# emtiyaz/vmp-for-svae

Measured on AMD Instinct MI355X. Metric: vmp_step_datapoints_per_sec, higher is better.
Workload: dtype f32

## Files before the change

### vmp-for-svae_amd/csrc/vmp_mix.hip

```cpp
#include "vmp_common.h"
#include "vmp_linalg.h"
#include <stdlib.h>
#include <type_traits>

using namespace vmp;

namespace {

constexpr int TR = 64;
constexpr int LS = 68;
constexpr int MAX_NW = 8;
constexpr int MAX_NW1 = 8;
constexpr int max_nw(int KT) { return KT == 1 ? MAX_NW1 : MAX_NW; }
constexpr int MAX_BLOCKS = 1024;

struct PassArgs {
    const float* x;
    const float* r_in;
    const float* u_in;
    const uint8_t* mask;
    const float* pivot;
    const float* pack;
    float* r_out;
    float* u_out;
    float* logr_out;
    double* partials;
    long long N;
    long long rpw;
    long long rpw_b;
    int K;
    int vec_ok;
    int par_reduce;
#ifdef VMP_DEBUG_TS
    long long* dbg_t;
#endif
};
#ifdef VMP_DEBUG_TS
#define PASS_TS(i) do { if (a.dbg_t && (blockIdx.x == 0 || blockIdx.x == 100) && (threadIdx.x & 63) == 0) { a.dbg_t[(blockIdx.x ? 64 : 0) + (threadIdx.x >> 6) * 8 + (i)] = clock64(); \
    if ((i) == 0 && threadIdx.x == 0) a.dbg_t[(blockIdx.x ? 64 : 0) + 7] = wall_clock64();           \
    if ((i) == 5 && threadIdx.x == 64) a.dbg_t[(blockIdx.x ? 64 : 0) + 8 + 7] = wall_clock64(); } } while (0)
#else
#define PASS_TS(i) do { } while (0)
#endif

#define VMP_DPP2(OP, CTRL)                                                   \
    "v_" OP "_f32_dpp %0, %0, %0 " CTRL " row_mask:0xf bank_mask:0xf\n\t"  \
    "v_" OP "_f32_dpp %1, %1, %1 " CTRL " row_mask:0xf bank_mask:0xf\n\t"  \
    "s_nop 0\n\t"
#define VMP_DPP2_FIRST(OP, CTRL)                                             \
    "v_" OP "_f32_dpp %0, %2, %2 " CTRL " row_mask:0xf bank_mask:0xf\n\t"  \
    "v_" OP "_f32_dpp %1, %3, %3 " CTRL " row_mask:0xf bank_mask:0xf\n\t"  \
    "s_nop 0\n\t"
__device__ __forceinline__ v2f row16_max2(v2f v) {
    float a, b;
    asm("s_nop 1\n\t" VMP_DPP2_FIRST("max", "row_ror:8") VMP_DPP2("max", "row_ror:4") VMP_DPP2("max", "row_ror:2")
        VMP_DPP2("max", "row_ror:1")
        : "=&v"(a), "=&v"(b) : "v"(v.x), "v"(v.y));
    return v2f{a, b};
}
__device__ __forceinline__ v2f row16_sum2(v2f v) {
    float a, b;
    asm("s_nop 1\n\t" VMP_DPP2_FIRST("add", "row_ror:8") VMP_DPP2("add", "row_ror:4") VMP_DPP2("add", "row_ror:2")
        VMP_DPP2("add", "row_ror:1")
        : "=&v"(a), "=&v"(b) : "v"(v.x), "v"(v.y));
    return v2f{a, b};
}

constexpr int MOM_TERMS = 3;
#ifndef VMP_MOM_FLUSH
#define VMP_MOM_FLUSH 2
#endif

template <int D, int KT, int FLAV>
__device__ __forceinline__ void pass_epilogue(const PassArgs& a, float* smem, const double (&dacc)[KT][Geo<D>::FT][4],
                                              const double (&dn)[KT][4], int lane, int wave, int nw) {
    using G = Geo<D>;
    constexpr int FT = G::FT;
    constexpr bool SMM = (FLAV == VMP_SMM);
    const int K = a.K;
    {
        __syncthreads();
        PASS_TS(3);
        double* sc = reinterpret_cast<double*>(smem);
        constexpr int SLAB = KT * (FT + 1) * 4 * WAVE;
        if (a.par_reduce) {
            double* mine = sc + wave * SLAB;
#pragma unroll
            for (int kt = 0; kt < KT; ++kt)
#pragma unroll
                for (int c = 0; c < 4; ++c) {
#pragma unroll
                    for (int ft = 0; ft < FT; ++ft) mine[((kt * (FT + 1) + ft) * 4 + c) * WAVE + lane] = dacc[kt][ft][c];
                    mine[((kt * (FT + 1) + FT) * 4 + c) * WAVE + lane] = SMM ? dn[kt][c] : dacc[kt][0][c];
                }
            __syncthreads();
            constexpr int EPT = 2, NWB = max_nw(KT);
            for (int e0 = threadIdx.x; e0 < SLAB; e0 += EPT * blockDim.x) {
                double vals[EPT][NWB];
#pragma unroll
                for (int q = 0; q < EPT; ++q) {
                    const int e = e0 + q * blockDim.x;
#pragma unroll
                    for (int w = 0; w < NWB; ++w) vals[q][w] = (e < SLAB && w < nw) ? sc[w * SLAB + e] : 0.0;
                }
#pragma unroll
                for (int q = 0; q < EPT; ++q) {
                    const int e = e0 + q * blockDim.x;
                    double t2 = vals[q][0];
#pragma unroll
                    for (int w = 1; w < NWB; ++w) t2 += vals[q][w];
                    if (e < SLAB) sc[e] = t2;
                }
            }
            __syncthreads();
        } else {
            for (int w = 0; w < nw; ++w) {
                if (wave == w) {
#pragma unroll
                    for (int kt = 0; kt < KT; ++kt)
#pragma unroll
                        for (int c = 0; c < 4; ++c) {
#pragma unroll
                            for (int ft = 0; ft < FT; ++ft) {
                                const int idx = ((kt * (FT + 1) + ft) * 4 + c) * WAVE + lane;
                                sc[idx] = (w == 0 ? 0.0 : sc[idx]) + dacc[kt][ft][c];
                            }
                            const int idn = ((kt * (FT + 1) + FT) * 4 + c) * WAVE + lane;
                            sc[idn] = (w == 0 ? 0.0 : sc[idn]) + (SMM ? dn[kt][c] : dacc[kt][0][c]);
                        }
                }
                __syncthreads();
            }
        }
        PASS_TS(4);
        constexpr int PX = G::PF + 1;
        double* out = a.partials;
        for (int e = threadIdx.x; e < KT * (FT + 1) * 4 * WAVE; e += blockDim.x) {
            const int l = e & 63, c = (e >> 6) & 3, tf = (e >> 8) % (FT + 1), kt = (e >> 8) / (FT + 1);
            const int k = kt * 16 + (l >> 4) * 4 + c;
            if (k >= K) continue;
            double* row = out + ((long long)k * MAX_BLOCKS + blockIdx.x) * PX;
            if (tf < FT) {
                const int f = tf * 16 + (l & 15);
                if (f < G::F) row[f] = sc[e];
            } else if ((l & 15) == 0) {
                row[G::F] = sc[e];
            }
        }
        if (wave == 0) {
            double ntot = 0.0;
#pragma unroll
            for (int kt = 0; kt < KT; ++kt) {
                const int k = kt * 16 + (lane & 15), l = ((k & 15) >> 2) * 16, c = k & 3;
                const double nk = (lane < 16 && k < K) ? sc[((kt * (FT + 1) + FT) * 4 + c) * WAVE + l] : 0.0;
#pragma unroll
                for (int j = 0; j < 16; ++j) ntot += readlane_d(nk, j);
            }
            for (int k = lane; k < K; k += WAVE) out[((long long)k * MAX_BLOCKS + blockIdx.x) * PX + G::PF] = ntot;
        }
        PASS_TS(5);
    }
}

template <int D, int KT, int FLAV, bool ESTEP, bool STATS, bool MASK>
__global__ __launch_bounds__(max_nw(KT) * WAVE) void pass_kernel(PassArgs a) {
    using G = Geo<D>;
    constexpr int FT = G::FT;
    constexpr bool SMM = (FLAV == VMP_SMM);
    extern __shared__ __attribute__((aligned(16))) float smem[];

    const int lane = threadIdx.x & 63, wave = threadIdx.x >> 6, nw = blockDim.x >> 6;
    const int K = a.K;
    PASS_TS(0);
#ifdef VMP_DEBUG_TS
    if (a.dbg_t && (blockIdx.x == 0 || blockIdx.x == 100) && (threadIdx.x & 63) == 0)
        a.dbg_t[(blockIdx.x ? 64 : 0) + (threadIdx.x >> 6) * 8 + 6] = __builtin_amdgcn_s_getreg((31 << 11) | 4);
#endif
    float* xl = smem + wave * (G::XROWS * LS);
    constexpr int ONE = D, ZERO = D + 1;
    xl[ONE * LS + lane] = 1.0f;
    xl[ZERO * LS + lane] = 0.0f;
    const int ppos = (lane & ~7) + 2 * (lane & 3) + ((lane >> 2) & 1);

    const bool vec = a.vec_ok != 0;
    long long lo, hi;
    if (a.rpw_b == a.rpw) {
        lo = ((long long)blockIdx.x * nw + wave) * a.rpw;
        hi = lo + a.rpw;
    } else {
        const int hw = nw >> 1;
        const long long base = (long long)blockIdx.x * hw * (a.rpw + a.rpw_b);
        lo = wave < hw ? base + wave * a.rpw : base + hw * a.rpw + (wave - hw) * a.rpw_b;
        hi = lo + (wave < hw ? a.rpw : a.rpw_b);
    }
    if (hi > a.N) hi = a.N;
    float xr[D];
    {
        const long long n = lo + lane;
#pragma unroll
        for (int j = 0; j < D; ++j) xr[j] = 0.f;
        if (n < hi) load_row<D>(a.x + n * D, xr, vec);
    }
    const int i16 = lane & 15, kk = lane >> 4;
    float pv[D];
    {
        const float* __restrict__ pp = a.pivot ? a.pivot : a.x;
        const bool hasp = a.pivot != nullptr;
#pragma unroll
        for (int j = 0; j < D; ++j) { const float v = pp[j]; pv[j] = hasp ? v : 0.f; }
    }

    constexpr int MP = (D + 1) / 2, WP = (G::TRI + 1) / 2;
    v2f pm2[KT][MP], pw2[KT][WP], pch[KT];
    float pua[KT], pub[KT];
    if constexpr (ESTEP) {
#pragma unroll
        for (int kt = 0; kt < KT; ++kt) {
            const int k = kt * 16 + i16;
            const bool on = k < K;
// ... 234 lines not shown
#pragma unroll
                    for (int ft = 0; ft < FT; ++ft) {
                        split_bf16<MOM_TERMS>(fa[ft] * fb[ft], t3);
#pragma unroll
                        for (int t = 0; t < 3; ++t) Bs[ft][t][u] = t3[t];
                    }
                }
            };
            using std::integral_constant;
            const bool full = (K == 16 * KT) && (n0 + 32 <= trows);
            if (full) {
                group(integral_constant<bool, true>{}, integral_constant<int, 0>{});
                group(integral_constant<bool, true>{}, integral_constant<int, 1>{});
                group(integral_constant<bool, true>{}, integral_constant<int, 2>{});
                group(integral_constant<bool, true>{}, integral_constant<int, 3>{});
            } else {
                group(integral_constant<bool, false>{}, integral_constant<int, 0>{});
                group(integral_constant<bool, false>{}, integral_constant<int, 1>{});
                group(integral_constant<bool, false>{}, integral_constant<int, 2>{});
                group(integral_constant<bool, false>{}, integral_constant<int, 3>{});
            }

            if constexpr (STATS) {
                bf16x8 b[FT][3];
#pragma unroll
                for (int ft = 0; ft < FT; ++ft)
#pragma unroll
                    for (int t = 0; t < 3; ++t)
                        b[ft][t] = __builtin_bit_cast(bf16x8, u32x4{Bs[ft][t][0], Bs[ft][t][1], Bs[ft][t][2], Bs[ft][t][3]});
#pragma unroll
                for (int kt = 0; kt < KT; ++kt) {
                    bf16x8 av[3], rv[3];
#pragma unroll
                    for (int t = 0; t < 3; ++t) {
                        av[t] = __builtin_bit_cast(bf16x8, u32x4{As[kt][t][0], As[kt][t][1], As[kt][t][2], As[kt][t][3]});
                        if constexpr (SMM) rv[t] = __builtin_bit_cast(bf16x8, u32x4{Rs[kt][t][0], Rs[kt][t][1], Rs[kt][t][2], Rs[kt][t][3]});
                    }
#pragma unroll
                    for (int ta = 0; ta < MOM_TERMS; ++ta) {
#pragma unroll
                        for (int tb = 0; tb + ta < MOM_TERMS; ++tb) {
#pragma unroll
                            for (int ft = 0; ft < FT; ++ft) {
                                if (ta + tb == 0) acc[kt][ft] = __builtin_amdgcn_mfma_f32_16x16x32_bf16(av[ta], b[ft][tb], acc[kt][ft], 0, 0, 0);
                                else acs[kt][ft] = __builtin_amdgcn_mfma_f32_16x16x32_bf16(av[ta], b[ft][tb], acs[kt][ft], 0, 0, 0);
                            }
                        }
                        if constexpr (SMM) {
                            if (ta == 0) nacc[kt] = __builtin_amdgcn_mfma_f32_16x16x32_bf16(rv[ta], b[0][0], nacc[kt], 0, 0, 0);
                            else nacs[kt] = __builtin_amdgcn_mfma_f32_16x16x32_bf16(rv[ta], b[0][0], nacs[kt], 0, 0, 0);
                        }
                    }
                }
            }
        }

        if constexpr (STATS) {
            if (((row0 - lo) / TR) % VMP_MOM_FLUSH == VMP_MOM_FLUSH - 1 || row0 + TR >= hi) {
#pragma unroll
                for (int kt = 0; kt < KT; ++kt) {
#pragma unroll
                    for (int c = 0; c < 4; ++c) {
                        if constexpr (SMM) dn[kt][c] += (double)nacc[kt][c] + (double)nacs[kt][c];
#pragma unroll
                        for (int ft = 0; ft < FT; ++ft) dacc[kt][ft][c] += (double)acc[kt][ft][c] + (double)acs[kt][ft][c];
                    }
                    nacc[kt] = f32x4{0.f, 0.f, 0.f, 0.f};
                    nacs[kt] = f32x4{0.f, 0.f, 0.f, 0.f};
#pragma unroll
                    for (int ft = 0; ft < FT; ++ft) { acc[kt][ft] = f32x4{0.f, 0.f, 0.f, 0.f}; acs[kt][ft] = f32x4{0.f, 0.f, 0.f, 0.f}; }
                }
            }
        }
        __builtin_amdgcn_wave_barrier();
    }

    PASS_TS(2);
    if constexpr (STATS) pass_epilogue<D, KT, FLAV>(a, smem, dacc, dn, lane, wave, nw);
}


constexpr int AIS = 36;

struct FinArgs {
    const double* partials;
    const double* stats_in;
    int nblk, K, flavour, src, do_post;
    const float *alpha0, *beta0, *m0, *C0, *v0, *kappa;
    const float* pivot;
    float *alpha, *beta, *m, *C, *v, *xbar, *S, *pi, *pack;
    double* pack64;
    double* stats_out;
    double* peer[VMP_EXCH_MAX_RANKS];
    int nranks, rank;
    unsigned long long iter;
    int* status;
#ifdef VMP_DEBUG_TS
    long long* dbg_t;
#endif
};

#ifdef VMP_DEBUG_TS
#define FIN_TS(i) do { if (a.dbg_t && blockIdx.x == 0 && tid == 0) { a.dbg_t[i] = clock64(); if ((i) == 0) a.dbg_t[6] = wall_clock64(); if ((i) == 5) a.dbg_t[7] = wall_clock64(); } } while (0)
#else
#define FIN_TS(i) do { } while (0)
#endif

template <int D>
__device__ void finalize_block(const FinArgs& a, const int k, const int tid, const int nthreads);

template <int D> constexpr int xdl_wave_floats() { return Geo<D>::XROWS * LS + TR * AIS; }

template <int D, int FLAV, bool STATS, int MT = 3>
__device__ __forceinline__ void pass_xdl_body(const PassArgs& a) {
    using G = Geo<D>;
    constexpr int FT = G::FT, KT = 1;
    constexpr bool SMM = (FLAV == VMP_SMM);
    constexpr int DP = (D + 1) / 2;
    extern __shared__ __attribute__((aligned(16))) float smem[];
    const int lane = threadIdx.x & 63, wave = threadIdx.x >> 6, nw = blockDim.x >> 6;
    const int K = a.K;
    PASS_TS(0);
    float* xl = smem + wave * xdl_wave_floats<D>();
    unsigned* ai = reinterpret_cast<unsigned*>(xl + G::XROWS * LS);
    constexpr int ONE = D, ZERO = D + 1;
    const int ppos = (lane & ~15) + 4 * (lane & 3) + ((lane >> 2) & 3);

    const bool vec = a.vec_ok != 0;
    long long lo, hi;
    if (a.rpw_b == a.rpw) {
        lo = ((long long)blockIdx.x * nw + wave) * a.rpw;
        hi = lo + a.rpw;
    } else {
        const int hw = nw >> 1;
        const long long base = (long long)blockIdx.x * hw * (a.rpw + a.rpw_b);
        lo = wave < hw ? base + wave * a.rpw : base + hw * a.rpw + (wave - hw) * a.rpw_b;
        hi = lo + (wave < hw ? a.rpw : a.rpw_b);
    }
    if (hi > a.N) hi = a.N;
    float xr[D];
    {
        const long long n = lo + lane;
#pragma unroll
        for (int j = 0; j < D; ++j) xr[j] = 0.f;
        if (n < hi) load_row<D>(a.x + n * D, xr, vec);
    }
    const int i16 = lane & 15, kk = lane >> 4;
    float pv[D];
    {
        const float* __restrict__ pp = a.pivot ? a.pivot : a.x;
        const bool hasp = a.pivot != nullptr;
#pragma unroll
        for (int j = 0; j < D; ++j) { const float v = pp[j]; pv[j] = hasp ? v : 0.f; }
    }

    constexpr int NS = D < 4 ? D : 4;
    constexpr int NB = D > 4 ? D - 4 : 0;
    constexpr int QK = 3 * NS + 4 * NB, QS = QK | 1;
    static_assert(16 * QS * 4 <= xdl_wave_floats<D>(), "the operand image must fit the LDS of a one-wave launch");
    u32x4 Bsm[NS], B1[NB > 0 ? NB : 1], B2[NB > 0 ? NB : 1];
    v2f pch;
    float pua, pub;
    {
        const bool on = i16 < K;
        const float* __restrict__ pc = a.pack + (on ? i16 : 0) * G::PACK + D + G::TRI;
        const float c0 = pc[0], c1 = pc[1], c2 = pc[2], c3 = pc[3];
        pch.x = on ? c0 : -INFINITY;
        pch.y = on ? c1 : 0.f;
        pua = on ? c2 : 0.f;
        pub = on ? c3 : 1.f;
    }
    {
        u32x4* img = reinterpret_cast<u32x4*>(smem);
        for (int it = threadIdx.x; it < 16 * D; it += blockDim.x) {
            const int k = it / D, i = it - k * D;
            const bool on = k < K;
            const float* __restrict__ p = a.pack + (on ? k : 0) * G::PACK;
            const int tri = i * (i + 1) / 2;
            float mr[D], wr[D];
#pragma unroll
            for (int j = 0; j < D; ++j) { mr[j] = p[j]; wr[j] = p[D + tri + j]; }
            double bi = 0.0;
#pragma unroll
            for (int j = 0; j < D; ++j)
                if (j <= i) bi -= (double)wr[j] * ((double)mr[j] - (double)pv[j]);
            unsigned tb[3];
            split_bf16<3>(v2f{(float)bi, 0.f}, tb);
            const unsigned bias0 = (tb[0] & 0xffffu) | (tb[1] << 16), bias1 = tb[2] & 0xffffu;
            unsigned th[4] = {0u, 0u, 0u, 0u}, tm[4] = {0u, 0u, 0u, 0u}, tl[4] = {0u, 0u, 0u, 0u};
#pragma unroll
            for (int q = 0; q < DP; ++q) {
                const int j0 = 2 * q, j1 = 2 * q + 1;
                const float wa = j0 <= i ? wr[j0] : 0.f;
                const float wb = (j1 <= i && j1 < D) ? wr[j1 < D ? j1 : 0] : 0.f;
                unsigned t3[3];
                split_bf16<3>(v2f{wa, wb}, t3);
                th[q] = t3[0]; tm[q] = t3[1]; tl[q] = t3[2];
            }
            const u32x4 zero = u32x4{0u, 0u, 0u, 0u};
            const u32x4 bias = on ? u32x4{bias0, bias1, 0u, 0u} : zero;
            if (i < NS) {
                u32x4* o = img + k * QS + 3 * i;
                o[0] = on ? u32x4{th[0], th[1], tm[0], tm[1]} : zero;
                o[1] = on ? u32x4{th[0], th[1], tl[0], tl[1]} : zero;
                o[2] = bias;
            } else {
                u32x4* o = img + k * QS + 3 * NS + 4 * (i - 4);
                o[0] = on ? u32x4{th[0], th[1], th[2], th[3]} : zero;
                o[1] = on ? u32x4{tm[0], tm[1], tm[2], tm[3]} : zero;
                o[2] = on ? u32x4{tl[0], tl[1], tl[2], tl[3]} : zero;
                o[3] = bias;
            }
        }
        __syncthreads();
        const u32x4* q = img + i16 * QS;
        const int s0 = kk == 1 ? 1 : (kk == 3 ? 2 : 0);
#pragma unroll
        for (int i = 0; i < NS; ++i) Bsm[i] = q[3 * i + s0];
        if constexpr (NB > 0) {
            const int s1 = kk == 1 ? 3 : (kk == 2 ? 1 : 0), s2 = kk == 0 ? 2 : (kk == 1 ? 0 : 1);
#pragma unroll
            for (int ib = 0; ib < NB; ++ib) {
                B1[ib] = q[3 * NS + 4 * ib + s1];
                const u32x4 w2 = q[3 * NS + 4 * ib + s2];
                B2[ib] = kk == 3 ? u32x4{0u, 0u, 0u, 0u} : w2;
            }
        }
        __syncthreads();
    }
    xl[ONE * LS + lane] = 1.0f;
    xl[ZERO * LS + lane] = 0.0f;
    {
        u32x4 ones = u32x4{0x3F803F80u, 0x00003F80u, 0u, 0u}, zeros = u32x4{0u, 0u, 0u, 0u};
        *reinterpret_cast<u32x4*>(ai + lane * AIS + 12) = ones;
        *reinterpret_cast<u32x4*>(ai + lane * AIS + 16) = zeros;
    }
    const int rho = 4 * (i16 & 3) + (i16 >> 2);
    const int offA1 = rho * AIS + (kk == 1 ? 12 : (kk == 3 ? 4 : 0));
    const int offA2 = rho * AIS + (kk == 0 ? 0 : (kk == 1 ? 8 : (kk == 2 ? 4 : 16)));
    const int offA3 = rho * AIS + (kk == 3 ? 12 : 20 + 4 * kk);

    int offA[FT], offB[FT];
#pragma unroll
    for (int ft = 0; ft < FT; ++ft) {
        const int f = ft * 16 + i16;
        int ra = ZERO, rb = ZERO;
        if (f == 0) { ra = ONE; rb = ONE; }
        else if (f <= D) { ra = f - 1; rb = ONE; }
        else if (f < G::F) {
            int p = f - D - 1, d = 0;
            while (p >= D - d) { p -= D - d; ++d; }
            ra = d; rb = d + p;
        }
        offA[ft] = ra * LS + 4 * kk;
        offB[ft] = rb * LS + 4 * kk;
    }

    f32x4 acc[KT][FT], acs[KT][FT];
    double dacc[KT][FT][4];
    double dn[KT][4];
    float nsum = 0.f;
    double dnl = 0.0;
#pragma unroll
    for (int c = 0; c < 4; ++c) dn[0][c] = 0.0;
#pragma unroll
    for (int ft = 0; ft < FT; ++ft) {
        acc[0][ft] = f32x4{0.f, 0.f, 0.f, 0.f};
        acs[0][ft] = f32x4{0.f, 0.f, 0.f, 0.f};
#pragma unroll
        for (int c = 0; c < 4; ++c) dacc[0][ft][c] = 0.0;
    }

#ifdef VMP_DEBUG_TS
    asm volatile("" :: "v"(xr[0]), "v"(pv[0]), "v"(pch.x), "v"(Bsm[0][0]));
    asm volatile("s_waitcnt vmcnt(0)" ::: "memory");
#endif
    PASS_TS(1);
    for (long long row0 = lo; row0 < hi; row0 += TR) {
        const int trows = (hi - row0 < TR) ? (int)(hi - row0) : TR;
        {
            const bool valid = row0 + lane < hi;
            float xs[2 * DP];
#pragma unroll
            for (int j = 0; j < 2 * DP; ++j) xs[j] = (valid && j < D) ? xr[j < D ? j : 0] - pv[j < D ? j : 0] : 0.f;
#pragma unroll
            for (int j = 0; j < D; ++j) xl[j * LS + ppos] = xs[j];
            unsigned th[4] = {0u, 0u, 0u, 0u}, tm[4] = {0u, 0u, 0u, 0u}, tl[4] = {0u, 0u, 0u, 0u};
#pragma unroll
            for (int q = 0; q < DP; ++q) {
                unsigned t3[3];
                split_bf16<3>(v2f{xs[2 * q], xs[2 * q + 1]}, t3);
                th[q] = t3[0]; tm[q] = t3[1]; tl[q] = t3[2];
            }
            *reinterpret_cast<u32x4*>(ai + lane * AIS) = u32x4{th[0], th[1], th[2], th[3]};
            *reinterpret_cast<u32x4*>(ai + lane * AIS + 4) = u32x4{tm[0], tm[1], tm[2], tm[3]};
            *reinterpret_cast<u32x4*>(ai + lane * AIS + 8) = u32x4{tl[0], tl[1], tl[2], tl[3]};
            *reinterpret_cast<u32x4*>(ai + lane * AIS + 20) = u32x4{th[0], th[1], th[0], th[1]};
            *reinterpret_cast<u32x4*>(ai + lane * AIS + 24) = u32x4{tm[0], tm[1], th[0], th[1]};
            *reinterpret_cast<u32x4*>(ai + lane * AIS + 28) = u32x4{tl[0], tl[1], tm[0], tm[1]};
            const long long n2 = row0 + TR + lane;
#pragma unroll
            for (int j = 0; j < D; ++j) xr[j] = 0.f;
            if (n2 < hi) load_row<D>(a.x + n2 * D, xr, vec);
        }
        __builtin_amdgcn_wave_barrier();

        const long long tbase = (row0 + kk) * K + i16;
#pragma unroll 1
        for (int n0 = 0; n0 < trows; n0 += 32) {
            const bool full = (K == 16) && (n0 + 32 <= trows);
            auto body = [&](auto full_c) __attribute__((always_inline)) {
            constexpr bool FULL = decltype(full_c)::value;
            unsigned As[3][4], Bs[FT][3][4];
            auto subtile = [&](auto jj_c) __attribute__((always_inline)) {
                constexpr int jj = decltype(jj_c)::value;
                const int n16 = n0 + 16 * jj;
                if (!FULL && n16 >= trows) {
                    if constexpr (STATS) {
#pragma unroll
                        for (int t = 0; t < 3; ++t) {
                            As[t][2 * jj] = 0u; As[t][2 * jj + 1] = 0u;
#pragma unroll
                            for (int ft = 0; ft < FT; ++ft) { Bs[ft][t][2 * jj] = 0u; Bs[ft][t][2 * jj + 1] = 0u; }
                        }
                    }
                    return;
                }
                f32x4 y[D];
                {
                    const bf16x8 a3 = __builtin_bit_cast(bf16x8, *reinterpret_cast<const u32x4*>(ai + n16 * AIS + offA3));
#pragma unroll
                    for (int i = 0; i < NS; ++i)
                        y[i] = __builtin_amdgcn_mfma_f32_16x16x32_bf16(a3, __builtin_bit_cast(bf16x8, Bsm[i]), f32x4{0.f, 0.f, 0.f, 0.f}, 0, 0, 0);
                }
                if constexpr (NB > 0) {
                    const bf16x8 a1 = __builtin_bit_cast(bf16x8, *reinterpret_cast<const u32x4*>(ai + n16 * AIS + offA1));
                    const bf16x8 a2 = __builtin_bit_cast(bf16x8, *reinterpret_cast<const u32x4*>(ai + n16 * AIS + offA2));
#pragma unroll
                    for (int i = 0; i < NB; ++i)
                        y[4 + i] = __builtin_amdgcn_mfma_f32_16x16x32_bf16(a1, __builtin_bit_cast(bf16x8, B1[i]), f32x4{0.f, 0.f, 0.f, 0.f}, 0, 0, 0);
#pragma unroll
                    for (int i = 0; i < NB; ++i)
                        y[4 + i] = __builtin_amdgcn_mfma_f32_16x16x32_bf16(a2, __builtin_bit_cast(bf16x8, B2[i]), y[4 + i], 0, 0, 0);
                }
                f32x4 q4 = y[0] * y[0], q4b = f32x4{0.f, 0.f, 0.f, 0.f};
#pragma unroll
                for (int i = 1; i < D; ++i) {
                    if (i & 1) q4b = __builtin_elementwise_fma(y[i], y[i], q4b);
                    else q4 = __builtin_elementwise_fma(y[i], y[i], q4);
                }
                q4 += q4b;
                v2f lg[2], uu[2], rr[2], w[2];
#pragma unroll
                for (int h = 0; h < 2; ++h) {
                    const v2f qh = v2f{q4[2 * h], q4[2 * h + 1]};
                    lg[h] = pk_const_minus_scaled(qh, pch);
                    if constexpr (SMM) uu[h] = v2f{pua * __builtin_amdgcn_rcpf(qh.x + pub), pua * __builtin_amdgcn_rcpf(qh.y + pub)};
                }
#pragma unroll
                for (int h = 0; h < 2; ++h) {
                    const v2f mx = row16_max2(lg[h]);
                    lg[h] = v2f{__builtin_amdgcn_exp2f(lg[h].x - mx.x), __builtin_amdgcn_exp2f(lg[h].y - mx.y)};
                    const v2f ssum = row16_sum2(lg[h]);
                    v2f inv = v2f{__builtin_amdgcn_rcpf(ssum.x), __builtin_amdgcn_rcpf(ssum.y)};
                    if constexpr (!FULL) {
                        const bool va = row0 + n16 + 8 * h + kk < hi, vb = row0 + n16 + 8 * h + 4 + kk < hi;
                        inv = v2f{va ? inv.x : 0.f, vb ? inv.y : 0.f};
                    }
                    rr[h] = lg[h] * inv;
                    w[h] = SMM ? rr[h] * uu[h] : rr[h];
                }
#pragma unroll
                for (int v = 0; v < 4; ++v) {
                    const float rv = rr[v >> 1][v & 1];
                    if constexpr (FULL) {
                        float* __restrict__ ro = a.r_out + tbase + (long long)(n16 + 4 * v) * 16;
                        __builtin_nontemporal_store(rv, ro);
                        if constexpr (SMM) __builtin_nontemporal_store(uu[v >> 1][v & 1], a.u_out + tbase + (long long)(n16 + 4 * v) * 16);
                        if (a.logr_out) a.logr_out[tbase + (long long)(n16 + 4 * v) * 16] = logf(rv);
                    } else {
                        const bool sv = (row0 + n16 + 4 * v + kk < hi) && i16 < K;
                        const long long o = tbase + (long long)(n16 + 4 * v) * K;
                        if (sv) {
                            a.r_out[o] = rv;
                            if constexpr (SMM) a.u_out[o] = uu[v >> 1][v & 1];
                            if (a.logr_out) a.logr_out[o] = logf(rv);
                        }
                    }
                }
                if constexpr (STATS) {
                    unsigned t3[3];
#pragma unroll
                    for (int h = 0; h < 2; ++h) {
                        split_bf16<MT>(w[h], t3);
#pragma unroll
                        for (int t = 0; t < 3; ++t) As[t][2 * jj + h] = t3[t];
                    }
                    if constexpr (SMM) nsum += (rr[0].x + rr[0].y) + (rr[1].x + rr[1].y);
#pragma unroll
                    for (int ft = 0; ft < FT; ++ft) {
                        const f32x4 fa = *reinterpret_cast<const f32x4*>(&xl[offA[ft] + n16]);
                        const f32x4 fb = *reinterpret_cast<const f32x4*>(&xl[offB[ft] + n16]);
                        const f32x4 pr = fa * fb;
#pragma unroll
                        for (int h = 0; h < 2; ++h) {
                            split_bf16<MT>(v2f{pr[2 * h], pr[2 * h + 1]}, t3);
#pragma unroll
                            for (int t = 0; t < 3; ++t) Bs[ft][t][2 * jj + h] = t3[t];
                        }
                    }
                }
            };
            using std::integral_constant;
            subtile(integral_constant<int, 0>{});
            subtile(integral_constant<int, 1>{});

            if constexpr (STATS) {
                bf16x8 b[FT][3];
#pragma unroll
                for (int ft = 0; ft < FT; ++ft)
#pragma unroll
                    for (int t = 0; t < 3; ++t)
                        b[ft][t] = __builtin_bit_cast(bf16x8, u32x4{Bs[ft][t][0], Bs[ft][t][1], Bs[ft][t][2], Bs[ft][t][3]});
                bf16x8 av[3];
#pragma unroll
                for (int t = 0; t < 3; ++t) av[t] = __builtin_bit_cast(bf16x8, u32x4{As[t][0], As[t][1], As[t][2], As[t][3]});
#pragma unroll
                for (int ta = 0; ta < MT; ++ta) {
#pragma unroll
                    for (int tb = 0; tb + ta < MT; ++tb) {
#pragma unroll
                        for (int ft = 0; ft < FT; ++ft) {
                            if (ta + tb == 0) acc[0][ft] = __builtin_amdgcn_mfma_f32_16x16x32_bf16(av[ta], b[ft][tb], acc[0][ft], 0, 0, 0);
                            else acs[0][ft] = __builtin_amdgcn_mfma_f32_16x16x32_bf16(av[ta], b[ft][tb], acs[0][ft], 0, 0, 0);
                        }
                    }
                }
            }
            };
            if (full) body(std::integral_constant<bool, true>{});
            else body(std::integral_constant<bool, false>{});
        }

        if constexpr (STATS) {
            if (((row0 - lo) / TR) % VMP_MOM_FLUSH == VMP_MOM_FLUSH - 1 || row0 + TR >= hi) {
#pragma unroll
                for (int c = 0; c < 4; ++c) {
#pragma unroll
                    for (int ft = 0; ft < FT; ++ft) dacc[0][ft][c] += (double)acc[0][ft][c] + (double)acs[0][ft][c];
                }
                if constexpr (SMM) { dnl += (double)nsum; nsum = 0.f; }
#pragma unroll
                for (int ft = 0; ft < FT; ++ft) { acc[0][ft] = f32x4{0.f, 0.f, 0.f, 0.f}; acs[0][ft] = f32x4{0.f, 0.f, 0.f, 0.f}; }
            }
        }
        __builtin_amdgcn_wave_barrier();
    }

    PASS_TS(2);
    if constexpr (STATS && SMM) {
        double tot = dnl;
        {
            int lo = __double2loint(tot), hi = __double2hiint(tot);
            tot += __hiloint2double(__shfl_xor(hi, 32), __shfl_xor(lo, 32));
            lo = __double2loint(tot); hi = __double2hiint(tot);
            tot += __hiloint2double(__shfl_xor(hi, 16), __shfl_xor(lo, 16));
        }
#pragma unroll
        for (int c = 0; c < 4; ++c) {
            const int src = 4 * kk + c;
            const int lo = __shfl(__double2loint(tot), src), hi = __shfl(__double2hiint(tot), src);
            dn[0][c] = __hiloint2double(hi, lo);
        }
    }
    if constexpr (STATS) pass_epilogue<D, 1, FLAV>(a, smem, dacc, dn, lane, wave, nw);
}

template <int D, int FLAV, bool STATS, int MT = 3>
__global__ __launch_bounds__(MAX_NW1 * WAVE) void pass_xdl_kernel(PassArgs a) {
    pass_xdl_body<D, FLAV, STATS, MT>(a);
}

__device__ double digamma_d(double x) {
    double r = 0.0;
    while (x < 10.0) { r -= 1.0 / x; x += 1.0; }
    const double f = 1.0 / (x * x);
    return r + log(x) - 0.5 / x
           - f * (1.0 / 12 - f * (1.0 / 120 - f * (1.0 / 252 - f * (1.0 / 240 - f * (1.0 / 132 - f * (691.0 / 32760))))));
}

template <int D>
__device__ void write_pack(float* pack, int k, const double* m, const double* W ,
                           double c, double h, double ua, double ub) {
    using G = Geo<D>;
    float* p = pack + k * G::PACK;
    int idx = D;
    for (int j = 0; j < D; ++j) p[j] = (float)m[j];
    for (int i = 0; i < D; ++i)
        for (int j = 0; j <= i; ++j) p[idx++] = (float)W[i * D + j];
    const double LOG2E = 1.4426950408889634074;
    p[idx++] = (float)(c * LOG2E); p[idx++] = (float)(h * LOG2E); p[idx++] = (float)ua; p[idx++] = (float)ub;
}

__device__ __forceinline__ double fast_rsqrt_d(double x) {
    double y = __builtin_amdgcn_rsq(x);
    y = y * (1.5 - 0.5 * x * y * y);
    y = y * (1.5 - 0.5 * x * y * y);
    return y;
}

template <int D>
__device__ __forceinline__ void wave_chol_inverse(const double* A, int lane, double (&X)[D], double& sumlog, bool& ok) {
    double row[D], rd[D];
#pragma unroll
    for (int e = 0; e < D; ++e)
        row[e] = lane < D ? 0.5 * (A[lane * D + e] + A[e * D + lane]) : (e == lane ? 1.0 : 0.0);
    ok = true;
    double mydiag = 1.0;
#pragma unroll
    for (int j = 0; j < D; ++j) {
        double t = row[j];
#pragma unroll
        for (int p = 0; p < j; ++p) t -= row[p] * readlane_d(row[p], j);
        const double sj = readlane_d(t, j);
        ok = ok && (sj > 0.0);
        rd[j] = fast_rsqrt_d(sj);
        if (lane == j) mydiag = sj;
        row[j] = lane >= j ? t * rd[j] : 0.0;
    }
    double lg = lane < D ? 0.5 * log(mydiag) : 0.0;
    sumlog = 0.0;
#pragma unroll
    for (int j = 0; j < D; ++j) sumlog += readlane_d(lg, j);
#pragma unroll
    for (int i = 0; i < D; ++i) {
        double acc = (i == lane) ? 1.0 : 0.0;
#pragma unroll
        for (int p = 0; p < i; ++p) acc -= readlane_d(row[p], i) * X[p];
        X[i] = acc * rd[i];
    }
}

template <int D>
__device__ void estep_constants(int k, int flavour, double alpha_k, double alpha_sum, double beta_k, double v_k,
                                double logdetP, double kap, double& c, double& h, double& ua, double& ub, double& elp) {
    const double LOG2 = 0.69314718055994530942, PI = 3.14159265358979323846;
    elp = digamma_d(alpha_k) - digamma_d(alpha_sum);
    double sdg = 0.0;
    if (flavour == VMP_GMM) {
        for (int i = 0; i < D; ++i) sdg += digamma_d(0.5 * (v_k + 1.0 + i));
        const double ld = (logdetP > log(1e-20)) ? logdetP : 0.0;
        const double eld = sdg + D * LOG2 + ld;
        c = elp + 0.5 * eld - 0.5 * (D / beta_k);
        h = 0.5; ua = 1.0; ub = 1.0;
    } else {
        for (int i = 0; i < D; ++i) sdg += digamma_d(0.5 * (v_k + i));
        const double eld = sdg + D * LOG2 + logdetP;
        h = 0.5 * (D + kap);
        c = lgamma(0.5 * (D + kap)) - lgamma(0.5 * kap) - 0.5 * D * log(kap * PI) + elp + 0.5 * eld
            - h * (D / beta_k) + log(kap);
        ua = D + kap;
        ub = D / beta_k + kap;
    }
}

constexpr int FIN_THREADS = 1024;
constexpr int FIN_MAX_GROUPS = FIN_THREADS / 64;

__device__ __forceinline__ void st_pack(const FinArgs& a, int idx, double v) {
    a.pack[idx] = (float)v;
    if (a.pack64) a.pack64[idx] = v;
}

template <int D>
__device__ void finalize_block(const FinArgs& a, const int k, const int tid, const int nthreads) {
    using G = Geo<D>;
    __shared__ double part[FIN_MAX_GROUPS][64];
    __shared__ double st[G::SW];
    __shared__ double ntot;
    __shared__ double Ck[D * D], mk[D], sp[D + 4], scal[8];
    __shared__ double alpha0s[VMP_MAX_K];
    const int K = a.K;
    const int FIN_GROUPS = nthreads >> 6;
    const bool post = a.do_post != 0;
    const bool smm = a.flavour == VMP_SMM;
    const double beta0 = post ? (double)a.beta0[k] : 0.0, v0 = post ? (double)a.v0[k] : 0.0;
    const double alpha0 = post ? (double)a.alpha0[k] : 0.0;
    const double kap = (post && smm) ? (double)a.kappa[k] : 0.0;
    bool shifted = (a.src == 0) && (a.pivot != nullptr);
    double m0d = 0.0, m0e = 0.0, C0de = 0.0, cd = 0.0, ce = 0.0;
    if (tid < D * D) {
        const int d = tid / D, e = tid % D;
        if (post) { m0d = a.m0[k * D + d]; m0e = a.m0[k * D + e]; C0de = a.C0[(k * D + d) * D + e]; }
        if (shifted) { cd = a.pivot[d]; ce = a.pivot[e]; }
    }
    if (post && tid < K) alpha0s[tid] = a.alpha0[tid];

    FIN_TS(0);
    if (a.src == 0) {
        constexpr int PX = G::PF + 1;
        const int f = tid & 63, g = tid >> 6;
        const double* __restrict__ mine = a.partials + (long long)k * MAX_BLOCKS * PX;
        for (int lg = g; lg < FIN_MAX_GROUPS; lg += FIN_GROUPS) {
            double s = 0.0;
            for (int b0 = lg; b0 < a.nblk; b0 += FIN_MAX_GROUPS * 16) {
                double v1[16];
                const int fc = f < PX ? f : PX - 1;
#pragma unroll
                for (int i = 0; i < 16; ++i) {
// ... 845 lines not shown
```

Measured before the change: 21.18 billion.

## Add specialized full-tile K=16 loop with fused 4-wide DPP softmax reductions

Splits the row loop into a fast path for full 64-row tiles when K==16, where both 32-row sub-bodies are unrolled with compile-time offsets and stride, and a generic tail loop. In the fast path the softmax max and sum reductions over the two half-tiles are interleaved into single 4-register DPP sequences, so independent DPP ops fill each other's hazard slots. The logr store is moved out of the per-element store loop, and the pivot is made wave-uniform via readfirstlane. This adds code size and register pressure.

```diff
diff --git a/vmp-for-svae_amd/csrc/vmp_mix.hip b/vmp-for-svae_amd/csrc/vmp_mix.hip
--- a/vmp-for-svae_amd/csrc/vmp_mix.hip
+++ b/vmp-for-svae_amd/csrc/vmp_mix.hip
@@ -65,6 +65,37 @@
         : "=&v"(a), "=&v"(b) : "v"(v.x), "v"(v.y));
     return v2f{a, b};
 }
+
+#define VMP_DPP4(OP, CTRL)                                                   \
+    "v_" OP "_f32_dpp %0, %0, %0 " CTRL " row_mask:0xf bank_mask:0xf\n\t"  \
+    "v_" OP "_f32_dpp %1, %1, %1 " CTRL " row_mask:0xf bank_mask:0xf\n\t"  \
+    "v_" OP "_f32_dpp %2, %2, %2 " CTRL " row_mask:0xf bank_mask:0xf\n\t"  \
+    "v_" OP "_f32_dpp %3, %3, %3 " CTRL " row_mask:0xf bank_mask:0xf\n\t"
+#define VMP_DPP4_FIRST(OP, CTRL)                                             \
+    "v_" OP "_f32_dpp %0, %4, %4 " CTRL " row_mask:0xf bank_mask:0xf\n\t"  \
+    "v_" OP "_f32_dpp %1, %5, %5 " CTRL " row_mask:0xf bank_mask:0xf\n\t"  \
+    "v_" OP "_f32_dpp %2, %6, %6 " CTRL " row_mask:0xf bank_mask:0xf\n\t"  \
+    "v_" OP "_f32_dpp %3, %7, %7 " CTRL " row_mask:0xf bank_mask:0xf\n\t"
+__device__ __forceinline__ void row16_max4(v2f v0, v2f v1, v2f& o0, v2f& o1) {
+    float a, b, c, d;
+    asm("s_nop 1\n\t" VMP_DPP4_FIRST("max", "row_ror:8") VMP_DPP4("max", "row_ror:4") VMP_DPP4("max", "row_ror:2")
+        VMP_DPP4("max", "row_ror:1")
+        : "=&v"(a), "=&v"(b), "=&v"(c), "=&v"(d) : "v"(v0.x), "v"(v0.y), "v"(v1.x), "v"(v1.y));
+    o0 = v2f{a, b};
+    o1 = v2f{c, d};
+}
+__device__ __forceinline__ void row16_sum4(v2f v0, v2f v1, v2f& o0, v2f& o1) {
+    float a, b, c, d;
+    asm("s_nop 1\n\t" VMP_DPP4_FIRST("add", "row_ror:8") VMP_DPP4("add", "row_ror:4") VMP_DPP4("add", "row_ror:2")
+        VMP_DPP4("add", "row_ror:1")
+        : "=&v"(a), "=&v"(b), "=&v"(c), "=&v"(d) : "v"(v0.x), "v"(v0.y), "v"(v1.x), "v"(v1.y));
+    o0 = v2f{a, b};
+    o1 = v2f{c, d};
+}
+
+#ifndef VMP_PASS_PIPE
+#define VMP_PASS_PIPE 3
+#endif
 
 constexpr int MOM_TERMS = 3;
 #ifndef VMP_MOM_FLUSH
@@ -605,6 +636,8 @@
         const bool hasp = a.pivot != nullptr;
 #pragma unroll
         for (int j = 0; j < D; ++j) { const float v = pp[j]; pv[j] = hasp ? v : 0.f; }
+#pragma unroll
+        for (int j = 0; j < D; ++j) pv[j] = __builtin_bit_cast(float, __builtin_amdgcn_readfirstlane(__builtin_bit_cast(int, pv[j])));
     }
 
     constexpr int NS = D < 4 ? D : 4;
@@ -729,10 +762,12 @@
     asm volatile("s_waitcnt vmcnt(0)" ::: "memory");
 #endif
     PASS_TS(1);
-    for (long long row0 = lo; row0 < hi; row0 += TR) {
-        const int trows = (hi - row0 < TR) ? (int)(hi - row0) : TR;
+    long long row0 = lo, tbase = 0;
+    int trows = TR;
+    auto stage = [&](auto whole_c) __attribute__((always_inline)) {
+        constexpr bool WHOLE = decltype(whole_c)::value;
         {
-            const bool valid = row0 + lane < hi;
+            const bool valid = WHOLE || row0 + lane < hi;
             float xs[2 * DP];
 #pragma unroll
             for (int j = 0; j < 2 * DP; ++j) xs[j] = (valid && j < D) ? xr[j < D ? j : 0] - pv[j < D ? j : 0] : 0.f;
@@ -757,157 +792,196 @@
             if (n2 < hi) load_row<D>(a.x + n2 * D, xr, vec);
         }
         __builtin_amdgcn_wave_barrier();
-
-        const long long tbase = (row0 + kk) * K + i16;
+        tbase = (row0 + kk) * (WHOLE ? 16 : K) + i16;
+    };
+    auto body = [&](auto full_c, auto n0_v) __attribute__((always_inline)) {
+        constexpr bool FULL = decltype(full_c)::value;
+        constexpr bool LINE = !std::is_same<decltype(n0_v), int>::value;
+        const int n0 = n0_v;
+        unsigned As[3][4], Bs[FT][3][4];
+        auto subtile = [&](auto jj_c) __attribute__((always_inline)) {
+            constexpr int jj = decltype(jj_c)::value;
+            const int n16 = n0 + 16 * jj;
+            if (!FULL && n16 >= trows) {
+                if constexpr (STATS) {
+#pragma unroll
+                    for (int t = 0; t < 3; ++t) {
+                        As[t][2 * jj] = 0u; As[t][2 * jj + 1] = 0u;
+#pragma unroll
+                        for (int ft = 0; ft < FT; ++ft) { Bs[ft][t][2 * jj] = 0u; Bs[ft][t][2 * jj + 1] = 0u; }
+                    }
+                }
+                return;
+            }
+            f32x4 y[D];
+            {
+                const bf16x8 a3 = __builtin_bit_cast(bf16x8, *reinterpret_cast<const u32x4*>(ai + n16 * AIS + offA3));
+#pragma unroll
+                for (int i = 0; i < NS; ++i)
+                    y[i] = __builtin_amdgcn_mfma_f32_16x16x32_bf16(a3, __builtin_bit_cast(bf16x8, Bsm[i]), f32x4{0.f, 0.f, 0.f, 0.f}, 0, 0, 0);
+            }
+            if constexpr (NB > 0) {
+                const bf16x8 a1 = __builtin_bit_cast(bf16x8, *reinterpret_cast<const u32x4*>(ai + n16 * AIS + offA1));
+                const bf16x8 a2 = __builtin_bit_cast(bf16x8, *reinterpret_cast<const u32x4*>(ai + n16 * AIS + offA2));
+#pragma unroll
+                for (int i = 0; i < NB; ++i)
+                    y[4 + i] = __builtin_amdgcn_mfma_f32_16x16x32_bf16(a1, __builtin_bit_cast(bf16x8, B1[i]), f32x4{0.f, 0.f, 0.f, 0.f}, 0, 0, 0);
+#pragma unroll
+                for (int i = 0; i < NB; ++i)
+                    y[4 + i] = __builtin_amdgcn_mfma_f32_16x16x32_bf16(a2, __builtin_bit_cast(bf16x8, B2[i]), y[4 + i], 0, 0, 0);
+            }
+            f32x4 q4 = y[0] * y[0], q4b = f32x4{0.f, 0.f, 0.f, 0.f};
+#pragma unroll
+            for (int i = 1; i < D; ++i) {
+                if (i & 1) q4b = __builtin_elementwise_fma(y[i], y[i], q4b);
+                else q4 = __builtin_elementwise_fma(y[i], y[i], q4);
+            }
+            q4 += q4b;
+            v2f lg[2], uu[2], rr[2], w[2];
+#pragma unroll
+            for (int h = 0; h < 2; ++h) {
+                const v2f qh = v2f{q4[2 * h], q4[2 * h + 1]};
+                lg[h] = pk_const_minus_scaled(qh, pch);
+                if constexpr (SMM) uu[h] = v2f{pua * __builtin_amdgcn_rcpf(qh.x + pub), pua * __builtin_amdgcn_rcpf(qh.y + pub)};
+            }
+            v2f mx[2], ssum[2];
+            if constexpr (LINE && VMP_PASS_PIPE >= 3) {
+                row16_max4(lg[0], lg[1], mx[0], mx[1]);
+#pragma unroll
+                for (int h = 0; h < 2; ++h) lg[h] = v2f{__builtin_amdgcn_exp2f(lg[h].x - mx[h].x), __builtin_amdgcn_exp2f(lg[h].y - mx[h].y)};
+                row16_sum4(lg[0], lg[1], ssum[0], ssum[1]);
+            } else {
+#pragma unroll
+                for (int h = 0; h < 2; ++h) {
+                    mx[h] = row16_max2(lg[h]);
+                    lg[h] = v2f{__builtin_amdgcn_exp2f(lg[h].x - mx[h].x), __builtin_amdgcn_exp2f(lg[h].y - mx[h].y)};
+                    ssum[h] = row16_sum2(lg[h]);
+                }
+            }
+#pragma unroll
+            for (int h = 0; h < 2; ++h) {
+                v2f inv = v2f{__builtin_amdgcn_rcpf(ssum[h].x), __builtin_amdgcn_rcpf(ssum[h].y)};
+                if constexpr (!FULL) {
+                    const bool va = row0 + n16 + 8 * h + kk < hi, vb = row0 + n16 + 8 * h + 4 + kk < hi;
+                    inv = v2f{va ? inv.x : 0.f, vb ? inv.y : 0.f};
+                }
+                rr[h] = lg[h] * inv;
+                w[h] = SMM ? rr[h] * uu[h] : rr[h];
+            }
+#pragma unroll
+            for (int v = 0; v < 4; ++v) {
+                const float rv = rr[v >> 1][v & 1];
+                if constexpr (FULL) {
+                    float* __restrict__ ro = a.r_out + tbase + (long long)(n16 + 4 * v) * 16;
+                    __builtin_nontemporal_store(rv, ro);
+                    if constexpr (SMM) __builtin_nontemporal_store(uu[v >> 1][v & 1], a.u_out + tbase + (long long)(n16 + 4 * v) * 16);
+                    if constexpr (!LINE)
+                        if (a.logr_out) a.logr_out[tbase + (long long)(n16 + 4 * v) * 16] = logf(rv);
+                } else {
+                    const bool sv = (row0 + n16 + 4 * v + kk < hi) && i16 < K;
+                    const long long o = tbase + (long long)(n16 + 4 * v) * K;
+                    if (sv) {
+                        a.r_out[o] = rv;
+                        if constexpr (SMM) a.u_out[o] = uu[v >> 1][v & 1];
+                        if (a.logr_out) a.logr_out[o] = logf(rv);
+                    }
+                }
+            }
+            if constexpr (LINE) {
+                if (a.logr_out) {
+#pragma unroll
+                    for (int v = 0; v < 4; ++v) a.logr_out[tbase + (long long)(n16 + 4 * v) * 16] = logf(rr[v >> 1][v & 1]);
+                }
+            }
+            if constexpr (STATS) {
+                unsigned t3[3];
+#pragma unroll
+                for (int h = 0; h < 2; ++h) {
+                    split_bf16<MT>(w[h], t3);
+#pragma unroll
+                    for (int t = 0; t < 3; ++t) As[t][2 * jj + h] = t3[t];
+                }
+                if constexpr (SMM) nsum += (rr[0].x + rr[0].y) + (rr[1].x + rr[1].y);
+#pragma unroll
+                for (int ft = 0; ft < FT; ++ft) {
+                    const f32x4 fa = *reinterpret_cast<const f32x4*>(&xl[offA[ft] + n16]);
+                    const f32x4 fb = *reinterpret_cast<const f32x4*>(&xl[offB[ft] + n16]);
+                    const f32x4 pr = fa * fb;
+#pragma unroll
+                    for (int h = 0; h < 2; ++h) {
+                        split_bf16<MT>(v2f{pr[2 * h], pr[2 * h + 1]}, t3);
+#pragma unroll
+                        for (int t = 0; t < 3; ++t) Bs[ft][t][2 * jj + h] = t3[t];
+                    }
+                }
+            }
+        };
+        using std::integral_constant;
+        subtile(integral_constant<int, 0>{});
+        subtile(integral_constant<int, 1>{});
+
+        if constexpr (STATS) {
+            bf16x8 b[FT][3];
+#pragma unroll
+            for (int ft = 0; ft < FT; ++ft)
+#pragma unroll
+                for (int t = 0; t < 3; ++t)
+                    b[ft][t] = __builtin_bit_cast(bf16x8, u32x4{Bs[ft][t][0], Bs[ft][t][1], Bs[ft][t][2], Bs[ft][t][3]});
+            bf16x8 av[3];
+#pragma unroll
+            for (int t = 0; t < 3; ++t) av[t] = __builtin_bit_cast(bf16x8, u32x4{As[t][0], As[t][1], As[t][2], As[t][3]});
+#pragma unroll
+            for (int ta = 0; ta < MT; ++ta) {
+#pragma unroll
+                for (int tb = 0; tb + ta < MT; ++tb) {
+#pragma unroll
+                    for (int ft = 0; ft < FT; ++ft) {
+                        if (ta + tb == 0) acc[0][ft] = __builtin_amdgcn_mfma_f32_16x16x32_bf16(av[ta], b[ft][tb], acc[0][ft], 0, 0, 0);
+                        else acs[0][ft] = __builtin_amdgcn_mfma_f32_16x16x32_bf16(av[ta], b[ft][tb], acs[0][ft], 0, 0, 0);
+                    }
+                }
+            }
+        }
+    };
+
+    auto flush = [&]() __attribute__((always_inline)) {
+        if constexpr (STATS) {
+            if (((row0 - lo) / TR) % VMP_MOM_FLUSH == VMP_MOM_FLUSH - 1 || row0 + TR >= hi) {
+#pragma unroll
+                for (int c = 0; c < 4; ++c) {
+#pragma unroll
+                    for (int ft = 0; ft < FT; ++ft) dacc[0][ft][c] += (double)acc[0][ft][c] + (double)acs[0][ft][c];
+                }
+                if constexpr (SMM) { dnl += (double)nsum; nsum = 0.f; }
+#pragma unroll
+                for (int ft = 0; ft < FT; ++ft) { acc[0][ft] = f32x4{0.f, 0.f, 0.f, 0.f}; acs[0][ft] = f32x4{0.f, 0.f, 0.f, 0.f}; }
+            }
+        }
+        __builtin_amdgcn_wave_barrier();
+    };
+
+    using std::integral_constant;
+    if (K == 16) {
+        for (; row0 + TR <= hi; row0 += TR) {
+#if VMP_PASS_PIPE == 1
+            asm volatile("s_waitcnt vmcnt(0)" ::: "memory");
+#endif
+            stage(integral_constant<bool, true>{});
+            body(integral_constant<bool, true>{}, integral_constant<int, 0>{});
+            body(integral_constant<bool, true>{}, integral_constant<int, 32>{});
+            flush();
+        }
+    }
+    for (; row0 < hi; row0 += TR) {
+        trows = (hi - row0 < TR) ? (int)(hi - row0) : TR;
+        stage(integral_constant<bool, false>{});
 #pragma unroll 1
         for (int n0 = 0; n0 < trows; n0 += 32) {
             const bool full = (K == 16) && (n0 + 32 <= trows);
-            auto body = [&](auto full_c) __attribute__((always_inline)) {
-            constexpr bool FULL = decltype(full_c)::value;
-            unsigned As[3][4], Bs[FT][3][4];
-            auto subtile = [&](auto jj_c) __attribute__((always_inline)) {
-                constexpr int jj = decltype(jj_c)::value;
-                const int n16 = n0 + 16 * jj;
-                if (!FULL && n16 >= trows) {
-                    if constexpr (STATS) {
-#pragma unroll
-                        for (int t = 0; t < 3; ++t) {
-                            As[t][2 * jj] = 0u; As[t][2 * jj + 1] = 0u;
-#pragma unroll
-                            for (int ft = 0; ft < FT; ++ft) { Bs[ft][t][2 * jj] = 0u; Bs[ft][t][2 * jj + 1] = 0u; }
-                        }
-                    }
-                    return;
-                }
-                f32x4 y[D];
-                {
-                    const bf16x8 a3 = __builtin_bit_cast(bf16x8, *reinterpret_cast<const u32x4*>(ai + n16 * AIS + offA3));
-#pragma unroll
-                    for (int i = 0; i < NS; ++i)
-                        y[i] = __builtin_amdgcn_mfma_f32_16x16x32_bf16(a3, __builtin_bit_cast(bf16x8, Bsm[i]), f32x4{0.f, 0.f, 0.f, 0.f}, 0, 0, 0);
-                }
-                if constexpr (NB > 0) {
-                    const bf16x8 a1 = __builtin_bit_cast(bf16x8, *reinterpret_cast<const u32x4*>(ai + n16 * AIS + offA1));
-                    const bf16x8 a2 = __builtin_bit_cast(bf16x8, *reinterpret_cast<const u32x4*>(ai + n16 * AIS + offA2));
-#pragma unroll
-                    for (int i = 0; i < NB; ++i)
-                        y[4 + i] = __builtin_amdgcn_mfma_f32_16x16x32_bf16(a1, __builtin_bit_cast(bf16x8, B1[i]), f32x4{0.f, 0.f, 0.f, 0.f}, 0, 0, 0);
-#pragma unroll
-                    for (int i = 0; i < NB; ++i)
-                        y[4 + i] = __builtin_amdgcn_mfma_f32_16x16x32_bf16(a2, __builtin_bit_cast(bf16x8, B2[i]), y[4 + i], 0, 0, 0);
-                }
-                f32x4 q4 = y[0] * y[0], q4b = f32x4{0.f, 0.f, 0.f, 0.f};
-#pragma unroll
-                for (int i = 1; i < D; ++i) {
-                    if (i & 1) q4b = __builtin_elementwise_fma(y[i], y[i], q4b);
-                    else q4 = __builtin_elementwise_fma(y[i], y[i], q4);
-                }
-                q4 += q4b;
-                v2f lg[2], uu[2], rr[2], w[2];
-#pragma unroll
-                for (int h = 0; h < 2; ++h) {
-                    const v2f qh = v2f{q4[2 * h], q4[2 * h + 1]};
-                    lg[h] = pk_const_minus_scaled(qh, pch);
-                    if constexpr (SMM) uu[h] = v2f{pua * __builtin_amdgcn_rcpf(qh.x + pub), pua * __builtin_amdgcn_rcpf(qh.y + pub)};
-                }
-#pragma unroll
-                for (int h = 0; h < 2; ++h) {
-                    const v2f mx = row16_max2(lg[h]);
-                    lg[h] = v2f{__builtin_amdgcn_exp2f(lg[h].x - mx.x), __builtin_amdgcn_exp2f(lg[h].y - mx.y)};
-                    const v2f ssum = row16_sum2(lg[h]);
-                    v2f inv = v2f{__builtin_amdgcn_rcpf(ssum.x), __builtin_amdgcn_rcpf(ssum.y)};
-                    if constexpr (!FULL) {
-                        const bool va = row0 + n16 + 8 * h + kk < hi, vb = row0 + n16 + 8 * h + 4 + kk < hi;
-                        inv = v2f{va ? inv.x : 0.f, vb ? inv.y : 0.f};
-                    }
-                    rr[h] = lg[h] * inv;
-                    w[h] = SMM ? rr[h] * uu[h] : rr[h];
-                }
-#pragma unroll
-                for (int v = 0; v < 4; ++v) {
-                    const float rv = rr[v >> 1][v & 1];
-                    if constexpr (FULL) {
-                        float* __restrict__ ro = a.r_out + tbase + (long long)(n16 + 4 * v) * 16;
-                        __builtin_nontemporal_store(rv, ro);
-                        if constexpr (SMM) __builtin_nontemporal_store(uu[v >> 1][v & 1], a.u_out + tbase + (long long)(n16 + 4 * v) * 16);
-                        if (a.logr_out) a.logr_out[tbase + (long long)(n16 + 4 * v) * 16] = logf(rv);
-                    } else {
-                        const bool sv = (row0 + n16 + 4 * v + kk < hi) && i16 < K;
-                        const long long o = tbase + (long long)(n16 + 4 * v) * K;
-                        if (sv) {
-                            a.r_out[o] = rv;
-                            if constexpr (SMM) a.u_out[o] = uu[v >> 1][v & 1];
-                            if (a.logr_out) a.logr_out[o] = logf(rv);
-                        }
-                    }
-                }
-                if constexpr (STATS) {
-                    unsigned t3[3];
-#pragma unroll
-                    for (int h = 0; h < 2; ++h) {
-                        split_bf16<MT>(w[h], t3);
-#pragma unroll
-                        for (int t = 0; t < 3; ++t) As[t][2 * jj + h] = t3[t];
-                    }
-                    if constexpr (SMM) nsum += (rr[0].x + rr[0].y) + (rr[1].x + rr[1].y);
-#pragma unroll
-                    for (int ft = 0; ft < FT; ++ft) {
-                        const f32x4 fa = *reinterpret_cast<const f32x4*>(&xl[offA[ft] + n16]);
-                        const f32x4 fb = *reinterpret_cast<const f32x4*>(&xl[offB[ft] + n16]);
-                        const f32x4 pr = fa * fb;
-#pragma unroll
-                        for (int h = 0; h < 2; ++h) {
-                            split_bf16<MT>(v2f{pr[2 * h], pr[2 * h + 1]}, t3);
-#pragma unroll
-                            for (int t = 0; t < 3; ++t) Bs[ft][t][2 * jj + h] = t3[t];
-                        }
-                    }
-                }
-            };
-            using std::integral_constant;
-            subtile(integral_constant<int, 0>{});
-            subtile(integral_constant<int, 1>{});
-
-            if constexpr (STATS) {
-                bf16x8 b[FT][3];
-#pragma unroll
-                for (int ft = 0; ft < FT; ++ft)
-#pragma unroll
-                    for (int t = 0; t < 3; ++t)
-                        b[ft][t] = __builtin_bit_cast(bf16x8, u32x4{Bs[ft][t][0], Bs[ft][t][1], Bs[ft][t][2], Bs[ft][t][3]});
-                bf16x8 av[3];
-#pragma unroll
-                for (int t = 0; t < 3; ++t) av[t] = __builtin_bit_cast(bf16x8, u32x4{As[t][0], As[t][1], As[t][2], As[t][3]});
-#pragma unroll
-                for (int ta = 0; ta < MT; ++ta) {
-#pragma unroll
-                    for (int tb = 0; tb + ta < MT; ++tb) {
-#pragma unroll
-                        for (int ft = 0; ft < FT; ++ft) {
-                            if (ta + tb == 0) acc[0][ft] = __builtin_amdgcn_mfma_f32_16x16x32_bf16(av[ta], b[ft][tb], acc[0][ft], 0, 0, 0);
-                            else acs[0][ft] = __builtin_amdgcn_mfma_f32_16x16x32_bf16(av[ta], b[ft][tb], acs[0][ft], 0, 0, 0);
-                        }
-                    }
-                }
-            }
-            };
-            if (full) body(std::integral_constant<bool, true>{});
-            else body(std::integral_constant<bool, false>{});
-        }
-
-        if constexpr (STATS) {
-            if (((row0 - lo) / TR) % VMP_MOM_FLUSH == VMP_MOM_FLUSH - 1 || row0 + TR >= hi) {
-#pragma unroll
-                for (int c = 0; c < 4; ++c) {
-#pragma unroll
-                    for (int ft = 0; ft < FT; ++ft) dacc[0][ft][c] += (double)acc[0][ft][c] + (double)acs[0][ft][c];
-                }
-                if constexpr (SMM) { dnl += (double)nsum; nsum = 0.f; }
-#pragma unroll
-                for (int ft = 0; ft < FT; ++ft) { acc[0][ft] = f32x4{0.f, 0.f, 0.f, 0.f}; acs[0][ft] = f32x4{0.f, 0.f, 0.f, 0.f}; }
-            }
-        }
-        __builtin_amdgcn_wave_barrier();
+            if (full) body(integral_constant<bool, true>{}, n0);
+            else body(integral_constant<bool, false>{}, n0);
+        }
+        flush();
     }
 
     PASS_TS(2);
```

Result: faster. 23.10 billion, median of 6 (+9.1%).
